# dog-qiuqiu/Yolo-FastestV2

Hardware: AMD Instinct MI355X
Metric: images/sec at 352x352 bs=256 per GPU (forward+decode+NMS) (higher is better)
Workload: dtype f32 tensors; contractions fp16x3 (two-term fp16 split operands on v_mfma_f32_16x16x32_f16, fp32 accumulate); depthwise/BN/ReLU/decode/NMS fp32 VALU; 1 GPU

## Files before the change

### include/yfv2.h

```cpp
#ifndef YFV2_H
#define YFV2_H

#include <stdint.h>

#ifdef __cplusplus
extern "C" {
#endif

#define YFV2_ABI_VERSION 7
#define YFV2_API __attribute__((visibility("default")))
#define YFV2_MAX_DET 300

typedef enum yfv2_status {
  YFV2_OK = 0,
  YFV2_ERR_ARG = -1,
  YFV2_ERR_CONFIG = -2,
  YFV2_ERR_DEVICE = -3,
  YFV2_ERR_WEIGHTS = -4,
  YFV2_ERR_STATE = -5,
  YFV2_ERR_BATCH = -6,
  YFV2_ERR_RANGE = -7
} yfv2_status;

typedef struct yfv2_ctx* yfv2_handle;
// ... 169 lines not shown

YFV2_API int yfv2_train_bind(yfv2_handle h, const yfv2_tensor_desc* tensors, int32_t n, const yfv2_tensor_desc* grads, int32_t ng);
YFV2_API int yfv2_train_forward(yfv2_handle h, const float* x, int32_t B, float* const out6[6], void* stream);
YFV2_API int yfv2_train_backward(yfv2_handle h, const float* const grad6[6], void* stream);
YFV2_API int yfv2_sgd_step(yfv2_handle h, float* param, const float* grad, float* momentum_buf, int64_t n, float lr, float momentum,
                           float weight_decay, int32_t first_step, void* stream);
typedef struct yfv2_sgd_item {
  float* param; const float* grad; float* momentum_buf;
  int64_t n;
  int32_t first_step; int32_t reserved;
} yfv2_sgd_item;
YFV2_API int yfv2_sgd_step_multi(yfv2_handle h, const yfv2_sgd_item* items, int32_t n_items, float lr, float momentum, float weight_decay,
                                 void* stream);


YFV2_API int32_t yfv2_num_rows(yfv2_handle h);
YFV2_API int32_t yfv2_num_stages(yfv2_handle h);

YFV2_API int yfv2_stage_info(yfv2_handle h, int32_t i, char* name, int32_t name_cap, double* flops_per_image,
                    double* bytes_per_image, double* external_bytes_per_image);
YFV2_API int yfv2_stage_kernel(yfv2_handle h, int32_t i, char* name, int32_t name_cap);

YFV2_API int yfv2_profile_forward(yfv2_handle h, const float* x, int32_t B, float* const out6[6], int32_t iters,
                         float* ms, void* stream);

YFV2_API int yfv2_clock_probe_begin(yfv2_handle h, int32_t workgroups, float milliseconds, int32_t busy, void* stream);
YFV2_API int yfv2_clock_probe_end(yfv2_handle h, double out[6], void* stream);

YFV2_API int yfv2_debug_repeat_step(yfv2_handle h, const float* x, int32_t B, float* const out6[6], int32_t step, int32_t iters, void* stream);

YFV2_API int yfv2_debug_post(yfv2_handle h, const float* const out6[6], int32_t B, float conf_thres, double iou_thres,
                             float* dets, int32_t* idx, int32_t* count, void* stream);

YFV2_API int64_t yfv2_debug_activation(yfv2_handle h, int32_t which, int32_t B, float* host_dst, int64_t cap);

YFV2_API int64_t yfv2_debug_train_relu_output(yfv2_handle h, const char* conv_name, float* host_dst, int64_t capacity);

YFV2_API int yfv2_debug_plan_dryrun(const yfv2_config* cfg, const yfv2_tensor_desc* tensors, int32_t n, int32_t* n_steps, int64_t* blob_floats);
YFV2_API int yfv2_debug_plan_dryrun_ex(const yfv2_config* cfg, const yfv2_plan* plan, const yfv2_tensor_desc* tensors, int32_t n, int32_t* n_steps,
                                       int64_t* blob_floats);
YFV2_API int64_t yfv2_debug_plan_image(const yfv2_config* cfg, const yfv2_tensor_desc* tensors, int32_t n, int32_t step, char* name,
                                       int32_t name_cap, float* dst, int64_t cap);
YFV2_API int64_t yfv2_debug_plan_image_ex(const yfv2_config* cfg, const yfv2_plan* plan, const yfv2_tensor_desc* tensors, int32_t n, int32_t step,
                                          char* name, int32_t name_cap, float* dst, int64_t cap);
YFV2_API int yfv2_debug_plan_c2_label(const yfv2_config* cfg, const yfv2_tensor_desc* tensors, int32_t n, int32_t* label);

#ifdef __cplusplus
}
#endif
#endif
```

### yolo_fastestv2_amd/_lib.py

```python
import ctypes as C
import os

_HERE = os.path.dirname(os.path.abspath(__file__))
LIB_PATH = os.environ.get("YFV2_LIB") or os.path.join(_HERE, "libyfv2.so")
ABI_VERSION = 7
MAX_DET = 300

OK, ERR_ARG, ERR_CONFIG, ERR_DEVICE, ERR_WEIGHTS, ERR_STATE, ERR_BATCH, ERR_RANGE = 0, -1, -2, -3, -4, -5, -6, -7


class Config(C.Structure):
    _fields_ = [("classes", C.c_int32), ("anchor_num", C.c_int32), ("height", C.c_int32), ("width", C.c_int32),
                ("anchors", C.c_double * 12), ("max_batch", C.c_int32), ("device", C.c_int32)]


class Plan(C.Structure):
    _fields_ = [("struct_size", C.c_int32), ("fp32_matrix", C.c_int32), ("layer_by_layer", C.c_int32), ("post_two_launches", C.c_int32),
                ("front_two_launches", C.c_int32), ("towers_unpaired", C.c_int32), ("lanes", C.c_int32), ("trace", C.c_int32), ("trace_step", C.c_int32)]


PLAN_FIELDS = ("fp32_matrix", "layer_by_layer", "post_two_launches", "front_two_launches", "towers_unpaired", "lanes", "trace", "trace_step")


def make_plan(plan=None):
# ... 108 lines not shown
    "yfv2_detect_frames_yuv": (C.c_int, [C.c_void_p, C.POINTER(FrameYuv), C.c_int32, C.c_float, C.c_double, C.c_void_p, C.c_void_p,
                                         C.c_void_p, C.c_void_p]),
    "yfv2_detect_tiled_yuv": (C.c_int, [C.c_void_p, C.POINTER(FrameYuv), C.c_int32, C.POINTER(Tile), C.c_int32, C.c_float, C.c_double, C.c_double,
                                        C.c_int32, C.c_int32, C.c_void_p, C.c_void_p, C.c_void_p, C.c_void_p]),
    "yfv2_train_batch_frames_u8": (C.c_int, [C.c_void_p, C.POINTER(Frame), C.c_int32, C.POINTER(C.c_float), C.POINTER(C.c_float), C.c_void_p, C.c_void_p]),
    "yfv2_train_batch_frames_yuv": (C.c_int, [C.c_void_p, C.POINTER(FrameYuv), C.c_int32, C.POINTER(C.c_float), C.POINTER(C.c_float), C.c_void_p, C.c_void_p]),
    "yfv2_export_maps": (C.c_int, [C.c_void_p, C.POINTER(C.c_void_p), C.c_int32, C.c_void_p, C.c_void_p, C.c_void_p]),
    "yfv2_deploy_post": (C.c_int, [C.c_void_p, C.c_void_p, C.c_void_p, C.c_int32, C.c_void_p, C.c_float, C.c_float, C.c_void_p, C.c_void_p,
                                   C.c_int32, C.c_void_p]),
    "yfv2_deploy_dropped": (C.c_int, [C.c_void_p, C.POINTER(C.c_int32), C.c_void_p]),
    "yfv2_detect_deploy_frames_u8": (C.c_int, [C.c_void_p, C.POINTER(Frame), C.c_int32, C.c_float, C.c_float, C.c_void_p, C.c_void_p,
                                               C.c_int32, C.c_void_p]),
    "yfv2_anchor_kmeans": (C.c_int, [C.c_void_p, C.c_void_p, C.c_int64, C.c_void_p, C.c_int32, C.c_int32, C.c_void_p, C.c_void_p,
                                     C.POINTER(KmeansInfo), C.c_void_p]),
    "yfv2_debug_kmeans_group": (C.c_int, [C.c_void_p, C.c_int32]),
    "yfv2_ap_per_class": (C.c_int, [C.c_void_p, C.c_void_p, C.c_void_p, C.c_void_p, C.c_int64, C.c_void_p, C.c_int64, C.POINTER(ApResult), C.c_void_p]),
    "yfv2_ap_per_class_multi": (C.c_int, [C.c_void_p, C.c_void_p, C.c_void_p, C.c_void_p, C.c_int64, C.c_void_p, C.c_int64, C.c_int32,
                                          C.POINTER(ApResult), C.c_void_p]),
    "yfv2_debug_plan_dryrun": (C.c_int, [C.c_void_p, C.c_void_p, C.c_int32, C.POINTER(C.c_int32), C.POINTER(C.c_int64)]),
    "yfv2_debug_plan_dryrun_ex": (C.c_int, [C.c_void_p, C.POINTER(Plan), C.c_void_p, C.c_int32, C.POINTER(C.c_int32), C.POINTER(C.c_int64)]),
    "yfv2_debug_plan_image": (C.c_int64, [C.c_void_p, C.c_void_p, C.c_int32, C.c_int32, C.c_char_p, C.c_int32, C.c_void_p, C.c_int64]),
    "yfv2_debug_plan_image_ex": (C.c_int64, [C.c_void_p, C.POINTER(Plan), C.c_void_p, C.c_int32, C.c_int32, C.c_char_p, C.c_int32, C.c_void_p, C.c_int64]),
    "yfv2_debug_plan_c2_label": (C.c_int, [C.c_void_p, C.c_void_p, C.c_int32, C.POINTER(C.c_int32)]),
    "yfv2_num_rows": (C.c_int32, [C.c_void_p]),
    "yfv2_num_stages": (C.c_int32, [C.c_void_p]),
    "yfv2_stage_info": (C.c_int, [C.c_void_p, C.c_int32, C.c_char_p, C.c_int32, C.POINTER(C.c_double),
                                  C.POINTER(C.c_double), C.POINTER(C.c_double)]),
    "yfv2_stage_kernel": (C.c_int, [C.c_void_p, C.c_int32, C.c_char_p, C.c_int32]),
    "yfv2_profile_forward": (C.c_int, [C.c_void_p, C.c_void_p, C.c_int32, C.POINTER(C.c_void_p), C.c_int32,
                                       C.POINTER(C.c_float), C.c_void_p]),
    "yfv2_debug_repeat_step": (C.c_int, [C.c_void_p, C.c_void_p, C.c_int32, C.POINTER(C.c_void_p), C.c_int32, C.c_int32, C.c_void_p]),
    "yfv2_debug_post": (C.c_int, [C.c_void_p, C.POINTER(C.c_void_p), C.c_int32, C.c_float, C.c_double, C.c_void_p, C.c_void_p,
                                  C.c_void_p, C.c_void_p]),
    "yfv2_debug_activation": (C.c_int64, [C.c_void_p, C.c_int32, C.c_int32, C.c_void_p, C.c_int64]),
    "yfv2_debug_train_relu_output": (C.c_int64, [C.c_void_p, C.c_char_p, C.c_void_p, C.c_int64]),
}

_lib = None


def lib():
    global _lib
    if _lib is not None:
        return _lib
    if not os.path.exists(LIB_PATH):
        raise ImportError("%s is missing: the HIP extension has not been built (run __graft_entry__.build()); "
                          "yolo_fastestv2_amd has no CPU or PyTorch fallback" % LIB_PATH)
    L = C.CDLL(LIB_PATH)
    if not hasattr(L, "yfv2_abi_version"):
        raise ImportError("%s does not export yfv2_abi_version: not a libyfv2 build" % LIB_PATH)
    L.yfv2_abi_version.restype, L.yfv2_abi_version.argtypes = C.c_int, []
    if L.yfv2_abi_version() != ABI_VERSION:
        raise ImportError("libyfv2.so ABI %d != binding ABI %d: rebuild (__graft_entry__.build())" % (L.yfv2_abi_version(), ABI_VERSION))
    for name, (res, args) in _PROTOTYPES.items():
        if name.startswith("yfv2_debug_") and os.environ.get("YFV2_LIB") and not hasattr(L, name):
            continue
        fn = getattr(L, name)
        fn.restype = res
        fn.argtypes = args
    _lib = L
    return L


def last_error(handle=None):
    msg = lib().yfv2_last_error(handle)
    return msg.decode("utf-8", "replace") if msg else ""
# ... 6 lines not shown
```

### yolo_fastestv2_amd/csrc/yfv2_api.hip

```cpp
#include <algorithm>
#include <cstdio>

#include "yfv2_ctx.h"

void read_plan_switches(yfv2_ctx* h, const yfv2_plan* plan) {
  h->sw.plan = read_sized(plan);
  h->sw.bf6 = !h->sw.plan.fp32_matrix;
  h->postfuse = !h->sw.plan.post_two_launches;
  h->sw.front_wanted = !h->sw.plan.front_two_launches;
}

int run_plan(yfv2_ctx* h, const void* x, bool x_u8, int B, float* const out6[6], hipStream_t stream, hipEvent_t* ev, int only_step) {
  const RunCtx c{h->d_params, x, x_u8, B, out6, stream, h->sw.bf6, h->nonfinite.dev};
  std::string err;
  if (int rc = plan_run(h->plan, c, h->d_trace, h->trace_step, ev, only_step, &err)) return fail(h, rc, err);
  if (only_step < 0) { h->last_x = x; h->last_B = B; h->last_u8 = x_u8; }
  HIP_TRY(h, hipGetLastError());
  return YFV2_OK;
}

int check_call(yfv2_ctx* h, int B, bool need_weights) {
  if (!h) return fail(nullptr, YFV2_ERR_ARG, "null handle");
  if (B < 1 || B > h->cfg.max_batch)
    return fail(h, YFV2_ERR_BATCH, "batch " + std::to_string(B) + " outside [1, max_batch=" + std::to_string(h->cfg.max_batch) + "]");
// ... 116 lines not shown
  return YFV2_OK;
}

void** yfv2_ctx_train_slot(yfv2_ctx* h) { return h ? &h->train : nullptr; }
const yfv2_config* yfv2_ctx_config(yfv2_ctx* h) { return &h->cfg; }
int yfv2_ctx_fail(yfv2_ctx* h, int code, const char* msg) {
  g_tls_error = msg ? msg : "";
  if (h) h->err = g_tls_error;
  return code;
}

DecodeArgs decode_args(yfv2_ctx* h, const float* const out6[6], int32_t B) {
  DecodeArgs a{};
  for (int sc = 0; sc < 2; ++sc) {
    a.reg[sc] = out6[sc * 3 + 0];
    a.obj[sc] = out6[sc * 3 + 1];
    a.cls[sc] = out6[sc * 3 + 2];
    a.fh[sc] = h->fh[sc];
    a.fw[sc] = h->fw[sc];
    a.stride[sc] = (float)((double)h->cfg.height / (double)h->fh[sc]);
  }
  for (int i = 0; i < 12; ++i) a.anchors[i] = h->cfg.anchors[i];
  a.B = B;
  a.classes = h->cfg.classes;
  a.rows = h->rows;
  return a;
}

NmsArgs nms_args(const yfv2_ctx* h, const float* boxes, int compact, int32_t B, float conf_thres, double iou_thres, float* dets, int32_t* idx, int32_t* count) {
  NmsArgs a{};
  a.boxes = boxes; a.compact = compact; a.dets = dets; a.idx = idx; a.count = count;
  a.B = B; a.rows = h->rows; a.nc = h->cfg.classes;
  a.conf_thres = conf_thres; a.iou_thres = iou_thres;
  return a;
}

static const void* image_at(const yfv2_ctx* h, const void* x, bool x_u8, int off) {
  return static_cast<const char*>(x) + (size_t)off * 3 * h->cfg.height * h->cfg.width * (x_u8 ? 1 : sizeof(float));
}

extern "C" {

int yfv2_abi_version(void) { return YFV2_ABI_VERSION; }

const char* yfv2_last_error(yfv2_handle h) { return h ? h->err.c_str() : g_tls_error.c_str(); }

int yfv2_create(yfv2_handle* out, const yfv2_config* cfg) { return yfv2_create_ex(out, cfg, nullptr); }

int yfv2_create_ex(yfv2_handle* out, const yfv2_config* cfg, const yfv2_plan* plan) {
  if (!out || !cfg) return fail(nullptr, YFV2_ERR_ARG, "yfv2_create: null argument");
  *out = nullptr;
  int rows = 0;
  if (int rc = check_config(cfg, &rows)) return rc;

  int ndev = 0;
  if (hipGetDeviceCount(&ndev) != hipSuccess || ndev <= 0 || cfg->device < 0 || cfg->device >= ndev)
    return fail(nullptr, YFV2_ERR_DEVICE, "no usable HIP device (this library has no CPU fallback)");
  hipDeviceProp_t prop;
  if (hipGetDeviceProperties(&prop, cfg->device) != hipSuccess)
    return fail(nullptr, YFV2_ERR_DEVICE, "hipGetDeviceProperties failed");
  if (std::strncmp(prop.gcnArchName, "gfx950", 6) != 0)
    return fail(nullptr, YFV2_ERR_DEVICE, std::string("device is ") + prop.gcnArchName + ", this library is built for gfx950 (MI355X) only");

  yfv2_ctx* h = new yfv2_ctx();
  h->in_lane = g_creating_lane;
  DeviceGuard guard(cfg->device);
// ... 244 lines not shown
```

### yolo_fastestv2_amd/csrc/yfv2_api_debug.hip

```cpp
#include <algorithm>
#include <cstdio>
#include <variant>

#include "yfv2_ctx.h"

namespace {

struct DryRun {
  yfv2_ctx ctx;
  WeightPacker wp;
  int build(const yfv2_config* cfg, const yfv2_plan* plan, const yfv2_tensor_desc* tensors, int32_t n) {
    int rows = 0;
    if (int rc = check_config(cfg, &rows)) return rc;
    uintptr_t next = 0x100000000ull;
    auto fake = [&](yfv2_ctx* hh, Buf* b, size_t per_img) {
      b->per_img = per_img;
      b->p = reinterpret_cast<float*>(next);
      next += (per_img * sizeof(float) * (size_t)hh->cfg.max_batch + 4095) & ~(uintptr_t)4095;
      return (int)YFV2_OK;
    };
    setup_ctx(&ctx, cfg, rows, fake);
    read_plan_switches(&ctx, plan);
    return build_plan(&ctx, wp, tensors, n, nullptr);
  }
};

}

extern "C" {

int yfv2_debug_plan_dryrun(const yfv2_config* cfg, const yfv2_tensor_desc* tensors, int32_t n, int32_t* n_steps, int64_t* blob_floats) {
  return yfv2_debug_plan_dryrun_ex(cfg, nullptr, tensors, n, n_steps, blob_floats);
}

int yfv2_debug_plan_dryrun_ex(const yfv2_config* cfg, const yfv2_plan* plan, const yfv2_tensor_desc* tensors, int32_t n, int32_t* n_steps, int64_t* blob_floats) {
  if (!cfg || !tensors || n <= 0) return fail(nullptr, YFV2_ERR_ARG, "yfv2_debug_plan_dryrun: bad argument");
  DryRun d;
  if (int rc = d.build(cfg, plan, tensors, n)) return rc;
  for (const Step& st : d.ctx.plan.steps)
    if (step_image(st) > d.wp.blob.size()) return fail(nullptr, YFV2_ERR_WEIGHTS, "step '" + st.name + "': image offset outside the blob");
  if (n_steps) *n_steps = (int32_t)d.ctx.plan.steps.size();
  if (blob_floats) *blob_floats = (int64_t)d.wp.blob.size();
  return YFV2_OK;
}

int64_t yfv2_debug_plan_image(const yfv2_config* cfg, const yfv2_tensor_desc* tensors, int32_t n, int32_t step, char* name, int32_t name_cap,
                              float* dst, int64_t cap) {
  return yfv2_debug_plan_image_ex(cfg, nullptr, tensors, n, step, name, name_cap, dst, cap);
}

int64_t yfv2_debug_plan_image_ex(const yfv2_config* cfg, const yfv2_plan* plan, const yfv2_tensor_desc* tensors, int32_t n, int32_t step, char* name,
                                 int32_t name_cap, float* dst, int64_t cap) {
  if (!cfg || !tensors || n <= 0 || (step != -1 && (!dst || cap <= 0))) return fail(nullptr, YFV2_ERR_ARG, "yfv2_debug_plan_image: bad argument");
  DryRun d;
  if (int rc = d.build(cfg, plan, tensors, n)) return rc;
  const int job = step >= 1000 ? step / 1000 - 1 : -1;
  if (step >= 1000) step %= 1000;
  std::vector<Step> view = d.ctx.plan.steps;
  if (d.ctx.plan.front_fused) { view.insert(view.begin(), d.ctx.plan.stem_aside); view[1].name = std::get<S2PxStep>(view[1].kind).name_plain; }
  if (step == -1) return (int64_t)view.size();
  if (step < 0 || step >= (int32_t)view.size()) return fail(nullptr, YFV2_ERR_ARG, "yfv2_debug_plan_image: step out of range");
  const TowerStep* tw = std::get_if<TowerStep>(&view[step].kind);
// ... 207 lines not shown
```

### yolo_fastestv2_amd/csrc/yfv2_internal.h

```cpp
#pragma once
#include <hip/hip_runtime.h>
#include <hip/hip_ext.h>
#include <stdint.h>

#include <atomic>

struct Yfv2LaunchProbe { hipEvent_t start = nullptr, stop = nullptr; int launches = 0; };
extern thread_local Yfv2LaunchProbe yfv2_launch_probe;
#define YFV2_LAUNCH(kernel, grid, block, lds, stream, ...)                                                                        \
  do {                                                                                                                             \
    Yfv2LaunchProbe& yfv2_lp_ = yfv2_launch_probe;                                                                                 \
    hipExtLaunchKernelGGL(kernel, grid, block, lds, stream, yfv2_lp_.launches++ == 0 ? yfv2_lp_.start : nullptr, yfv2_lp_.stop, 0, \
                          __VA_ARGS__);                                                                                            \
  } while (0)
struct Yfv2Device { int index, cus; };
inline Yfv2Device yfv2_device() {
  static std::atomic<int> cus_of[64];
  int dev = 0;
  if (hipGetDevice(&dev) != hipSuccess || dev < 0 || dev > 63) dev = 0;
  int cus = cus_of[dev].load(std::memory_order_relaxed);
  if (cus <= 0) { if (hipDeviceGetAttribute(&cus, hipDeviceAttributeMultiprocessorCount, dev) != hipSuccess || cus <= 0) cus = 256; cus_of[dev].store(cus, std::memory_order_relaxed); }
  return {dev, cus};
}
inline int yfv2_device_cus() { return yfv2_device().cus; }
// ... 162 lines not shown
  int B, H, W;
  long long* trace;
  int bf6;
  const float* img16;
  int chain;
  int* nonfinite;
};

struct DecodeArgs {
  const float* reg[2];
  const float* obj[2];
  const float* cls[2];
  float* boxes;
  float* cand;
  int B, classes;
  int fh[2], fw[2];
  float stride[2];
  double anchors[12];
  int rows;
};

struct NmsArgs {
  const float* boxes;
  int compact;
  float* dets;
  int32_t* idx;
  int32_t* count;
  const int32_t* classes;
  int n_classes;
  int B, rows, nc;
  float conf_thres;
  double iou_thres;
  long long* trace;
};

void yfv2_launch_stem(const StemArgs& a, hipStream_t s);
void yfv2_launch_stem16(const StemArgs& a, hipStream_t s);
bool yfv2_launch_pw(int K, int mode, const PwArgs& a, hipStream_t s);
int yfv2_pw_tiles(int K, int mode, int M);
bool yfv2_pw_presplit_supported(int K, int mode, int M);
bool yfv2_launch_dw(int ksize, int stride, const DwArgs& a, hipStream_t s);
int yfv2_block_s2_rows(int cin, int H, int W);
bool yfv2_launch_block_s2(int cin, const BlockS2Args& a, hipStream_t s);
bool yfv2_tower2_supported(int H, int W);
bool yfv2_launch_tower2(const TowerArgs& a, hipStream_t s);
bool yfv2_towerh_supported(int H, int W);
bool yfv2_towerh_multi(int H, int W);
bool yfv2_towerp_map(int H, int W);
void towerp_lane_patches(int H, int W, unsigned char (&tbl)[128]);
struct TowerJobs {
  TowerArgs j[4];
  int n;
  int par;
  int gpj;
  unsigned char lane_patch[128];
};
bool yfv2_launch_towerh(const TowerJobs& jobs, int mh_tiles, const Yfv2Device& dev, hipStream_t s);
struct StatsArgs {
  const float* dets;
  const int32_t* count;
  const float* targets;
  int32_t* tp;
  int32_t* overflow;
  int B, T;
  float iou_thres;
};
// ... 44 lines not shown
  double box_x, box_y;
};
void yfv2_launch_resize_frames(const ResizeFrame* frames, int B, int max_w, unsigned char* dst, int H, int W, hipStream_t s);
struct YuvCoef { int off, cy, cvr, cvg, cug, cub; };
struct ResizeFrameYuv {
  const unsigned char* y;
  const unsigned char* ca;
  const unsigned char* cb;
  long long pitch_y, pitch_c;
  int h, w;
  int px, py;
  int format;
  YuvCoef coef;
  double scale_x, scale_y;
};
size_t yfv2_resize_yuv_lds_bytes(int w, int W);
int yfv2_resize_yuv_max_width(int W);
YuvCoef yfv2_yuv_coef(int colour);
void yfv2_launch_resize_frames_yuv(const ResizeFrameYuv* frames, int B, int max_w, unsigned char* dst, int H, int W, hipStream_t s);
struct TrainFrame : ResizeFrame { float alpha, beta; };
struct TrainFrameYuv : ResizeFrameYuv { float alpha, beta; };
size_t yfv2_train_batch_lds_bytes(int SW, int W);
int yfv2_train_batch_max_width(int W);
size_t yfv2_train_batch_yuv_lds_bytes(int w, int W);
int yfv2_train_batch_yuv_max_width(int W);
void yfv2_launch_train_batch_frames(const TrainFrame* frames, int B, int max_w, float* dst , int H, int W, hipStream_t s);
void yfv2_launch_train_batch_frames_yuv(const TrainFrameYuv* frames, int B, int max_w, float* dst, int H, int W, hipStream_t s);
void yfv2_launch_frame_boxes(float* dets, const int32_t* count, const ResizeFrame* frames, int B, hipStream_t s);
void yfv2_launch_decode(const DecodeArgs& a, hipStream_t s);
void yfv2_launch_nms(const NmsArgs& a, hipStream_t s);
void yfv2_launch_decode_nms(const DecodeArgs& d, const NmsArgs& a, hipStream_t s);
bool yfv2_post_fusable(int classes, int rows);
int yfv2_nms_max_rows();
struct TileMergeArgs {
  const float* tile_dets;
  const int32_t* tile_count;
  const int32_t* table;
  int T, F;
  float* geo;
  float* meta;
  double thres;
  int metric;
  int max_out;
  float* dets;
  int32_t* src;
  int32_t* count;
};
void yfv2_launch_tile_merge(const TileMergeArgs& a, hipStream_t s);
struct ExportMapsArgs {
  const float* reg[2]; const float* obj[2]; const float* cls[2];
  float* map[2];
  int B, classes;
  int fh[2], fw[2];
};
void yfv2_launch_export_maps(const ExportMapsArgs& a, hipStream_t s);
struct DeployPostArgs {
  const float* map[2];
  const float* scale;
  int B, classes;
  int fh[2], fw[2];
  int stride[2];
  float anchors[12];
  int rows;
  float thresh, nms_thresh;
  int32_t* boxes;
  int32_t* count;
// ... 65 lines not shown
```

### yolo_fastestv2_amd/csrc/yfv2_post.hip

```cpp
#include "yfv2_device.h"


template <int J>
__device__ __forceinline__ int quad_xor(int v) {
  static_assert(J == 1 || J == 2, "quad_perm exchange inside four lanes");
  return __builtin_amdgcn_update_dpp(0, v, J == 1 ? 0xB1 : 0x4E, 0xF, 0xF, false);
}
template <int J> __device__ __forceinline__ float quad_xor(float v) { return __int_as_float(quad_xor<J>(__float_as_int(v))); }

template <bool SKIP = false, int MAXPER = 24>
__device__ __forceinline__ void yfv2_compact_row(const DecodeArgs& a, int b, int sc, int cc, int part, f32x4& r0, f32x4& r1,
                                                 float objl = 0.f, float skip_ct = 0.f) {
  const int fh = a.fh[sc], fw = a.fw[sc], hw = fh * fw;
  const int nc = a.classes;
  const int per = (nc + 3) >> 2;
  const int c_lo = part * per, c_hi = min(nc, c_lo + per);
  const int an = part < 3 ? part : 0;
  const float* cls = a.cls[sc] + (size_t)b * nc * hw;
  const float so = sigmoid_f32(SKIP ? objl : a.obj[sc][((size_t)b * 3 + an) * hw + cc]);
  float conf = 0.f;
  int cj = 0;
  int need = 1;
  if constexpr (SKIP) {
    need = so > skip_ct ? 1 : 0;
// ... 158 lines not shown
        float o[5];
        box_of(part, o);
        float* d = srow + part * rowlen;
#pragma unroll
        for (int k = 0; k < 5; ++k) d[k] = o[k];
      }
    }
    __syncthreads();
    float* dst = a.boxes + row0 * rowlen;
    const int n = ncell * 3 * rowlen;
    for (int i = tid; i < n; i += THREADS) dst[i] = stage[i];
  }
}

void yfv2_launch_decode(const DecodeArgs& a, hipStream_t s) {
  const int cells = a.classes <= 96 ? DEC_CELLS : 32;
  const int b0 = (a.fh[0] * a.fw[0] + cells - 1) / cells;
  const int b1 = (a.fh[1] * a.fw[1] + cells - 1) / cells;
  const size_t lds = (size_t)cells * 3 * (5 + a.classes) * sizeof(float);
  if (a.classes <= 96) {
    if (a.cand)
      YFV2_LAUNCH(decode_kernel<true>, dim3(a.B * (b0 + b1)), dim3(DEC_THREADS), 0, s, a, b0, b1);
    else
      YFV2_LAUNCH_LDS(yfv2_device(), decode_kernel<false>, YFV2_LDS_FULL, dim3(a.B * (b0 + b1)), dim3(DEC_THREADS), lds, s, a, b0, b1);
  } else {
    if (a.cand)
      YFV2_LAUNCH((decode_kernel<true, 64>), dim3(a.B * (b0 + b1)), dim3(4 * cells), 0, s, a, b0, b1);
    else
      YFV2_LAUNCH_LDS(yfv2_device(), (decode_kernel<false, 64>), YFV2_LDS_FULL, dim3(a.B * (b0 + b1)), dim3(4 * cells), lds, s, a, b0, b1);
  }
}
bool yfv2_post_fusable(int classes, int rows) { return classes <= 96 && rows <= 2048; }
int yfv2_nms_max_rows() { return 4096; }

constexpr int NMS_THREADS = 1024;
constexpr int NMS_NQ = NMS_THREADS / 64;
constexpr int NMS_CAP = 2048;
constexpr int NMS_MAX_DET = 300;

__device__ __forceinline__ unsigned xor_sel_mask() {
  const int l = (int)(threadIdx.x & 63);
  const bool s4 = __builtin_amdgcn_update_dpp(0, l, 0x124, 0xF, 0xF, false) == (l ^ 4);
  const auto p16 = __builtin_amdgcn_permlane16_swap(l, l, false, false);
  const auto p32 = __builtin_amdgcn_permlane32_swap(l, l, false, false);
  return (s4 ? 4u : 0u) | ((int)p16[0] == (l ^ 16) ? 16u : 0u) | ((int)p32[0] == (l ^ 32) ? 32u : 0u);
}
template <int J>
__device__ __forceinline__ unsigned xor_lane32(unsigned v, unsigned sel) {
  const int x = (int)v;
  if constexpr (J == 1 || J == 2) return (unsigned)quad_xor<J>(x);
  else if constexpr (J == 8) return (unsigned)__builtin_amdgcn_update_dpp(0, x, 0x128, 0xF, 0xF, false);
  else if constexpr (J == 4) {
    const int r4 = __builtin_amdgcn_update_dpp(0, x, 0x124, 0xF, 0xF, false), r12 = __builtin_amdgcn_update_dpp(0, x, 0x12C, 0xF, 0xF, false);
    return (unsigned)((sel & 4u) ? r4 : r12);
  } else if constexpr (J == 16) {
    const auto p = __builtin_amdgcn_permlane16_swap(x, x, false, false);
    return (unsigned)((sel & 16u) ? (int)p[0] : (int)p[1]);
  } else {
    static_assert(J == 32, "lane distance");
    const auto p = __builtin_amdgcn_permlane32_swap(x, x, false, false);
    return (unsigned)((sel & 32u) ? (int)p[0] : (int)p[1]);
  }
}
template <int J>
__device__ __forceinline__ unsigned long long xor_lane64(unsigned long long v, unsigned sel) {
  return ((unsigned long long)xor_lane32<J>((unsigned)(v >> 32), sel) << 32) | xor_lane32<J>((unsigned)v, sel);
}

template <int KPT>
__device__ __forceinline__ void bitonic_sort(unsigned long long* key, unsigned long long* key2, int np2, int tid) {
  const unsigned sel = xor_sel_mask();
// ... 36 lines not shown
      _Pragma("unroll") for (int r = 0; r < KPT; ++r) {                                     \
        const int i = tid + r * NMS_THREADS;                                                \
        k[r] = cx(k[r], xor_lane64<J>(k[r], sel), low == ((i & kk) == 0));                 \
      }                                                                                     \
    }
    YFV2_SORT_STEP(32) YFV2_SORT_STEP(16) YFV2_SORT_STEP(8) YFV2_SORT_STEP(4) YFV2_SORT_STEP(2) YFV2_SORT_STEP(1)
#undef YFV2_SORT_STEP
  }
  __syncthreads();
#pragma unroll
  for (int r = 0; r < KPT; ++r) { const int i = tid + r * NMS_THREADS; if (i < np2) key[i] = k[r]; }
  __syncthreads();
}

__device__ __forceinline__ unsigned conf_key(float c) {
  const unsigned u = __float_as_uint(c == 0.f ? 0.f : c);
  return (u & 0x80000000u) ? ~u : (u | 0x80000000u);
}

template <int SRC, int KPT = 2>
__global__ __launch_bounds__(NMS_THREADS) void nms_kernel(NmsArgs a, DecodeArgs dec) {
  constexpr bool COMPACT = SRC >= 1;
  constexpr int CAP = KPT * NMS_THREADS;
  static_assert(KPT == 2 || (KPT == 4 && SRC != 2), "two keys per thread, or four without the in-LDS decode");
  extern __shared__ __attribute__((aligned(16))) float crow[];
  __shared__ unsigned long long key[CAP];
  __shared__ __attribute__((aligned(16))) float geo[(KPT == 2 ? 7 : 5) * CAP];
  unsigned long long* const key2 = reinterpret_cast<unsigned long long*>(geo);
  float* const bx1 = geo + (KPT == 2 ? 2 * CAP : 0);
  float* const by1 = bx1 + CAP; float* const bx2 = by1 + CAP; float* const by2 = bx2 + CAP; float* const area = by2 + CAP;
  __shared__ unsigned char supp[CAP];
  __shared__ unsigned char cls_of_row[CAP];
  __shared__ int keep[NMS_MAX_DET];
  __shared__ float kx1[NMS_MAX_DET], kx2[NMS_MAX_DET];
  __shared__ unsigned long long pmask[NMS_NQ][64];
  __shared__ int n_cand, n_keep, n_obj;

  const int tid = threadIdx.x, b = blockIdx.x;
  const int rowlen = COMPACT ? 8 : 5 + a.nc;
  const float* img = SRC == 2 ? crow : a.boxes + (size_t)b * a.rows * rowlen;
  const float ct = a.conf_thres;
  YFV2_STAMP(0);
  if constexpr (SRC == 2) {
    constexpr int WC = 16;
    const int hw0 = dec.fh[0] * dec.fw[0], hw1 = dec.fh[1] * dec.fw[1];
    const int nw0 = (hw0 + WC - 1) / WC, nw = nw0 + (hw1 + WC - 1) / WC;
    const int wv = __builtin_amdgcn_readfirstlane(tid >> 6);
    const int part = tid & 3, an = part < 3 ? part : 0;
    auto obj_of = [&](int w) -> float {
      if (w >= nw) return 0.f;
      const int sc = w >= nw0 ? 1 : 0, hw = sc ? hw1 : hw0;
      const int cell = (w - (sc ? nw0 : 0)) * WC + ((tid & 63) >> 2);
      return dec.obj[sc][((size_t)b * 3 + an) * hw + (cell < hw ? cell : hw - 1)];
    };
    float ocur = obj_of(wv);
    for (int w = wv; w < nw; w += NMS_NQ) {
      const float onxt = obj_of(w + NMS_NQ);
      const int sc = w >= nw0 ? 1 : 0, hw = sc ? hw1 : hw0;
      const int row_base = sc ? 3 * hw0 : 0;
      const int cell = (w - (sc ? nw0 : 0)) * WC + ((tid & 63) >> 2);
      const bool ok = cell < hw;
      f32x4 r0, r1;
      yfv2_compact_row<true>(dec, b, sc, ok ? cell : hw - 1, part, r0, r1, ocur, ct);
      if (ok && part < 3) {
        float* d = crow + (size_t)(row_base + cell * 3 + part) * 8;
        *reinterpret_cast<f32x4*>(d) = r0;
        *reinterpret_cast<f32x4*>(d + 4) = r1;
// ... 70 lines not shown
    }
  }
  __syncthreads();
  YFV2_STAMP(2);
  const int n = n_cand;
  if (n == 0) {
    if (tid == 0) a.count[b] = 0;
    return;
  }

  int np2 = 1;
  while (np2 < n) np2 <<= 1;
  for (int i = n + tid; i < np2; i += NMS_THREADS) key[i] = 0ull;
  __syncthreads();
  if (np2 <= NMS_THREADS) bitonic_sort<1>(key, key2, np2, tid);
  else bitonic_sort<KPT>(key, key2, np2, tid);

  YFV2_STAMP(3);
  for (int i = tid; i < n; i += NMS_THREADS) {
    const unsigned row = 0xFFFFFFFFu - (unsigned)(key[i] & 0xFFFFFFFFull);
    const float* r = img + (size_t)row * rowlen;
    const float cx = r[0], cy = r[1], hw_ = __fdiv_rn(r[2], 2.0f), hh = __fdiv_rn(r[3], 2.0f);
    const float c = __fmul_rn((float)cls_of_row[row], 4096.0f);
    const float x1 = __fadd_rn(__fsub_rn(cx, hw_), c), y1 = __fadd_rn(__fsub_rn(cy, hh), c);
    const float x2 = __fadd_rn(__fadd_rn(cx, hw_), c), y2 = __fadd_rn(__fadd_rn(cy, hh), c);
    bx1[i] = x1; by1[i] = y1; bx2[i] = x2; by2[i] = y2;
    area[i] = __fmul_rn(__fsub_rn(x2, x1), __fsub_rn(y2, y1));
    supp[i] = 0;
  }
  __syncthreads();

  YFV2_STAMP(4);
  const bool thr_nonneg = a.iou_thres >= 0.0;
  auto overlaps = [&](int i, int j) -> bool {
    const float xx1 = fmaxf(bx1[i], bx1[j]), xx2 = fminf(bx2[i], bx2[j]);
    if (thr_nonneg && !(xx2 > xx1)) return false;
    const float yy1 = fmaxf(by1[i], by1[j]), yy2 = fminf(by2[i], by2[j]);
    const float w = fmaxf(0.0f, __fsub_rn(xx2, xx1)), h = fmaxf(0.0f, __fsub_rn(yy2, yy1));
    const float inter = __fmul_rn(w, h);
    const float ovr = __fdiv_rn(inter, __fsub_rn(__fadd_rn(area[i], area[j]), inter));
    return (double)ovr > a.iou_thres;
  };
  const int j = tid & 63, q = tid >> 6;
  long long t_tests = 0, t_walk = 0, t_bar = 0; int n_chunks = 0;
  const bool tr = a.trace && blockIdx.x == 0 && tid == 0;
  for (int c0 = 0; c0 < n; c0 += 64) {
    const int nk = n_keep;
    if (nk >= NMS_MAX_DET) break;
    const long long ts0 = tr ? (long long)__builtin_readcyclecounter() : 0;
    const int m = min(64, n - c0);
    unsigned long long bits = 0ull;
    {
      constexpr int KMAX = (NMS_MAX_DET + NMS_NQ - 1) / NMS_NQ;
      constexpr int PER = 64 / NMS_NQ;
      auto lane_f = [](float v, int l) { return __builtin_bit_cast(float, __builtin_amdgcn_readlane(__builtin_bit_cast(int, v), l)); };
      const int cj = c0 + j;
      const bool live = j < m;
      const float jx1 = live ? bx1[cj] : INFINITY, jx2 = live ? bx2[cj] : -INFINITY;
      const int kl = q + NMS_NQ * j;
      const bool kv = j < KMAX && kl < nk;
      const float rk1 = kv ? kx1[kl] : INFINITY, rk2 = kv ? kx2[kl] : -INFINITY;
      unsigned cand = 0u;
#pragma unroll
      for (int t = 0; t < KMAX; ++t) {
        const float a1 = lane_f(rk1, t), a2 = lane_f(rk2, t);
        if (q + NMS_NQ * t < nk && (!thr_nonneg || fminf(a2, jx2) > fmaxf(a1, jx1))) cand |= 1u << t;
      }
      unsigned icand = 0u;
#pragma unroll
      for (int c = 0; c < PER; ++c) {
        const int i = PER * q + c;
        const float a1 = lane_f(jx1, i), a2 = lane_f(jx2, i);
        if (i < j && (!thr_nonneg || fminf(a2, jx2) > fmaxf(a1, jx1))) icand |= 1u << c;
      }
      if (live) {
        while (cand) {
          const int t = __builtin_ctz(cand);
          cand &= cand - 1u;
          if (overlaps(keep[q + NMS_NQ * t], cj)) { supp[cj] = 1; break; }
        }
        while (icand) {
          const int c = __builtin_ctz(icand);
          icand &= icand - 1u;
          if (overlaps(c0 + PER * q + c, cj)) bits |= 1ull << (PER * q + c);
        }
      }
    }
    pmask[q][j] = bits;
    const long long ts1 = tr ? (long long)__builtin_readcyclecounter() : 0;
    __syncthreads();
    const long long ts2 = tr ? (long long)__builtin_readcyclecounter() : 0;
    if (tid < 64) {
      unsigned long long S = 0ull;
#pragma unroll
      for (int qq = 0; qq < NMS_NQ; ++qq) S |= pmask[qq][tid];
      const bool alive = tid < m && !supp[c0 + tid];
      const unsigned long long alive_mask = __ballot(alive);
      unsigned long long kmask = alive_mask;
      for (int it = 0; it < 64; ++it) {
        const unsigned long long k2 = __ballot(alive && !(S & kmask));
        if (k2 == kmask) break;
        kmask = k2;
      }
      if ((kmask >> tid) & 1ull) {
        const int pos = nk + __popcll(kmask & ((1ull << tid) - 1ull));
        if (pos < NMS_MAX_DET) { keep[pos] = c0 + tid; kx1[pos] = bx1[c0 + tid]; kx2[pos] = bx2[c0 + tid]; }
      }
      if (tid == 0) n_keep = min(NMS_MAX_DET, nk + __popcll(kmask));
    }
    const long long ts3 = tr ? (long long)__builtin_readcyclecounter() : 0;
    __syncthreads();
    if (tr) { const long long ts4 = (long long)__builtin_readcyclecounter(); t_tests += ts1 - ts0; t_walk += ts3 - ts2; t_bar += (ts2 - ts1) + (ts4 - ts3); ++n_chunks; }
  }
  if (tr) { a.trace[9] = n_chunks; a.trace[10] = t_tests; a.trace[11] = t_walk; a.trace[12] = t_bar; }
  __syncthreads();
  YFV2_STAMP(5);
  const int kept = n_keep;

  for (int k = tid; k < kept; k += NMS_THREADS) {
    const int i = keep[k];
    const unsigned long long kk = key[i];
    const unsigned row = 0xFFFFFFFFu - (unsigned)(kk & 0xFFFFFFFFull);
    const float* r = img + (size_t)row * rowlen;
    const float cx = r[0], cy = r[1], hw_ = __fdiv_rn(r[2], 2.0f), hh = __fdiv_rn(r[3], 2.0f);
    float* d = a.dets + ((size_t)b * NMS_MAX_DET + k) * 6;
    d[0] = __fsub_rn(cx, hw_); d[1] = __fsub_rn(cy, hh);
    d[2] = __fadd_rn(cx, hw_); d[3] = __fadd_rn(cy, hh);
    d[4] = COMPACT ? r[5] : __fmul_rn(r[5 + cls_of_row[row]], r[4]);
    d[5] = (float)cls_of_row[row];
    a.idx[(size_t)b * NMS_MAX_DET + k] = (int)row;
  }
  if (tid == 0) a.count[b] = kept;
  YFV2_STAMP(6);
  if (a.trace && blockIdx.x == 0 && tid == 0) { a.trace[7] = n; a.trace[8] = kept; }
}

void yfv2_launch_nms(const NmsArgs& a, hipStream_t s) {
  const DecodeArgs none{};
  if (a.rows <= NMS_CAP) {
// ... 170 lines not shown
```

Baseline: 463,400 images/s.

## Make NMS overlap tests wave-uniform with full kept-box arrays and a division-free reject

The NMS inner loop now keeps full kept-box coordinates and areas in LDS, laid out per wave, and tests them with wave-uniform scalar operands instead of divergent candidate walks. A conservative multiply-based test against a precomputed threshold skips the IoU division for pairs that clearly fall below the threshold. Within-chunk tests also compute full IoU for every lane instead of branching. The aim is to remove divergent loops and most divisions from the NMS critical path, at the cost of doing more uniform arithmetic per pair and a slightly larger LDS footprint.

```diff
diff --git a/include/yfv2.h b/include/yfv2.h
--- a/include/yfv2.h
+++ b/include/yfv2.h
@@ -225,6 +225,8 @@
 YFV2_API int yfv2_debug_post(yfv2_handle h, const float* const out6[6], int32_t B, float conf_thres, double iou_thres,
                              float* dets, int32_t* idx, int32_t* count, void* stream);
 
+YFV2_API int yfv2_debug_nms_reject(double iou_thres, float* c, float* c2);
+
 YFV2_API int64_t yfv2_debug_activation(yfv2_handle h, int32_t which, int32_t B, float* host_dst, int64_t cap);
 
 YFV2_API int64_t yfv2_debug_train_relu_output(yfv2_handle h, const char* conv_name, float* host_dst, int64_t capacity);
diff --git a/yolo_fastestv2_amd/_lib.py b/yolo_fastestv2_amd/_lib.py
--- a/yolo_fastestv2_amd/_lib.py
+++ b/yolo_fastestv2_amd/_lib.py
@@ -164,6 +164,7 @@
     "yfv2_debug_repeat_step": (C.c_int, [C.c_void_p, C.c_void_p, C.c_int32, C.POINTER(C.c_void_p), C.c_int32, C.c_int32, C.c_void_p]),
     "yfv2_debug_post": (C.c_int, [C.c_void_p, C.POINTER(C.c_void_p), C.c_int32, C.c_float, C.c_double, C.c_void_p, C.c_void_p,
                                   C.c_void_p, C.c_void_p]),
+    "yfv2_debug_nms_reject": (C.c_int, [C.c_double, C.POINTER(C.c_float), C.POINTER(C.c_float)]),
     "yfv2_debug_activation": (C.c_int64, [C.c_void_p, C.c_int32, C.c_int32, C.c_void_p, C.c_int64]),
     "yfv2_debug_train_relu_output": (C.c_int64, [C.c_void_p, C.c_char_p, C.c_void_p, C.c_int64]),
 }
diff --git a/yolo_fastestv2_amd/csrc/yfv2_api.hip b/yolo_fastestv2_amd/csrc/yfv2_api.hip
--- a/yolo_fastestv2_amd/csrc/yfv2_api.hip
+++ b/yolo_fastestv2_amd/csrc/yfv2_api.hip
@@ -172,6 +172,8 @@
   a.boxes = boxes; a.compact = compact; a.dets = dets; a.idx = idx; a.count = count;
   a.B = B; a.rows = h->rows; a.nc = h->cfg.classes;
   a.conf_thres = conf_thres; a.iou_thres = iou_thres;
+  float c;
+  a.rej_on = yfv2_nms_reject(iou_thres, &c, &a.rej_c2);
   return a;
 }
 
diff --git a/yolo_fastestv2_amd/csrc/yfv2_api_debug.hip b/yolo_fastestv2_amd/csrc/yfv2_api_debug.hip
--- a/yolo_fastestv2_amd/csrc/yfv2_api_debug.hip
+++ b/yolo_fastestv2_amd/csrc/yfv2_api_debug.hip
@@ -28,6 +28,14 @@
 }
 
 extern "C" {
+
+int yfv2_debug_nms_reject(double iou_thres, float* c, float* c2) {
+  float c_, c2_;
+  const int on = yfv2_nms_reject(iou_thres, &c_, &c2_);
+  if (c) *c = c_;
+  if (c2) *c2 = c2_;
+  return on;
+}
 
 int yfv2_debug_plan_dryrun(const yfv2_config* cfg, const yfv2_tensor_desc* tensors, int32_t n, int32_t* n_steps, int64_t* blob_floats) {
   return yfv2_debug_plan_dryrun_ex(cfg, nullptr, tensors, n, n_steps, blob_floats);
diff --git a/yolo_fastestv2_amd/csrc/yfv2_internal.h b/yolo_fastestv2_amd/csrc/yfv2_internal.h
--- a/yolo_fastestv2_amd/csrc/yfv2_internal.h
+++ b/yolo_fastestv2_amd/csrc/yfv2_internal.h
@@ -218,6 +218,8 @@
   float conf_thres;
   double iou_thres;
   long long* trace;
+  float rej_c2;
+  int rej_on;
 };
 
 void yfv2_launch_stem(const StemArgs& a, hipStream_t s);
@@ -328,6 +330,7 @@
 void yfv2_launch_decode_nms(const DecodeArgs& d, const NmsArgs& a, hipStream_t s);
 bool yfv2_post_fusable(int classes, int rows);
 int yfv2_nms_max_rows();
+int yfv2_nms_reject(double iou_thres, float* c, float* c2);
 struct TileMergeArgs {
   const float* tile_dets;
   const int32_t* tile_count;
diff --git a/yolo_fastestv2_amd/csrc/yfv2_post.hip b/yolo_fastestv2_amd/csrc/yfv2_post.hip
--- a/yolo_fastestv2_amd/csrc/yfv2_post.hip
+++ b/yolo_fastestv2_amd/csrc/yfv2_post.hip
@@ -214,11 +214,22 @@
 }
 bool yfv2_post_fusable(int classes, int rows) { return classes <= 96 && rows <= 2048; }
 int yfv2_nms_max_rows() { return 4096; }
+int yfv2_nms_reject(double iou_thres, float* c, float* c2) {
+  *c = 0.f; *c2 = 0.f;
+  if (!(iou_thres >= 0x1p-24 && iou_thres <= 1.0)) return 0;
+  auto fp32_at_most = [](double v) { float f = (float)v; return (double)f > v ? nextafterf(f, -INFINITY) : f; };
+  *c = fp32_at_most(iou_thres);
+  *c2 = fp32_at_most((double)*c * (1.0 - 0x1p-22));
+  return 1;
+}
 
 constexpr int NMS_THREADS = 1024;
 constexpr int NMS_NQ = NMS_THREADS / 64;
 constexpr int NMS_CAP = 2048;
 constexpr int NMS_MAX_DET = 300;
+#ifndef YFV2_NMS_UNIFORM
+#define YFV2_NMS_UNIFORM 1
+#endif
 
 __device__ __forceinline__ unsigned xor_sel_mask() {
   const int l = (int)(threadIdx.x & 63);
@@ -321,7 +332,8 @@
   __shared__ unsigned char supp[CAP];
   __shared__ unsigned char cls_of_row[CAP];
   __shared__ int keep[NMS_MAX_DET];
-  __shared__ float kx1[NMS_MAX_DET], kx2[NMS_MAX_DET];
+  constexpr int KMAX = (NMS_MAX_DET + NMS_NQ - 1) / NMS_NQ;
+  __shared__ float kx1[NMS_NQ * KMAX], ky1[NMS_NQ * KMAX], kx2[NMS_NQ * KMAX], ky2[NMS_NQ * KMAX], karea[NMS_NQ * KMAX];
   __shared__ unsigned long long pmask[NMS_NQ][64];
   __shared__ int n_cand, n_keep, n_obj;
 
@@ -458,59 +470,92 @@
 
   YFV2_STAMP(4);
   const bool thr_nonneg = a.iou_thres >= 0.0;
-  auto overlaps = [&](int i, int j) -> bool {
-    const float xx1 = fmaxf(bx1[i], bx1[j]), xx2 = fminf(bx2[i], bx2[j]);
-    if (thr_nonneg && !(xx2 > xx1)) return false;
-    const float yy1 = fmaxf(by1[i], by1[j]), yy2 = fminf(by2[i], by2[j]);
+  const bool rej_on = a.rej_on != 0;
+  const float rej_c2 = a.rej_c2;
+  auto vmax = [](auto a, float m) -> float {
+    float r;
+    if constexpr (__is_same(decltype(a), int)) asm("v_max_f32 %0, %1, %2" : "=v"(r) : "s"(a), "v"(m));
+    else asm("v_max_f32 %0, %1, %2" : "=v"(r) : "v"(a), "v"(m));
+    return r;
+  };
+  auto vmin = [](auto a, float m) -> float {
+    float r;
+    if constexpr (__is_same(decltype(a), int)) asm("v_min_f32 %0, %1, %2" : "=v"(r) : "s"(a), "v"(m));
+    else asm("v_min_f32 %0, %1, %2" : "=v"(r) : "v"(a), "v"(m));
+    return r;
+  };
+  auto pair = [&](auto ax1, auto ay1, auto ax2, auto ay2, float aarea, float mx1, float my1, float mx2, float my2, float marea, float& inter, float& uni) {
+    const float xx1 = vmax(ax1, mx1), xx2 = vmin(ax2, mx2);
+    const float yy1 = vmax(ay1, my1), yy2 = vmin(ay2, my2);
     const float w = fmaxf(0.0f, __fsub_rn(xx2, xx1)), h = fmaxf(0.0f, __fsub_rn(yy2, yy1));
-    const float inter = __fmul_rn(w, h);
-    const float ovr = __fdiv_rn(inter, __fsub_rn(__fadd_rn(area[i], area[j]), inter));
-    return (double)ovr > a.iou_thres;
+    inter = __fmul_rn(w, h);
+    uni = __fsub_rn(__fadd_rn(aarea, marea), inter);
   };
-  const int j = tid & 63, q = tid >> 6;
+  auto rejected = [&](float inter, float uni) -> bool { return rej_on && uni >= 0x1p-100f && uni < INFINITY && inter < __fmul_rn(rej_c2, uni); };
+  auto above = [&](float inter, float uni) -> bool { return (double)__fdiv_rn(inter, uni) > a.iou_thres; };
+  const int j = tid & 63, q = __builtin_amdgcn_readfirstlane(tid >> 6);
   long long t_tests = 0, t_walk = 0, t_bar = 0; int n_chunks = 0;
   const bool tr = a.trace && blockIdx.x == 0 && tid == 0;
   for (int c0 = 0; c0 < n; c0 += 64) {
-    const int nk = n_keep;
+    const int nk = __builtin_amdgcn_readfirstlane(n_keep);
     if (nk >= NMS_MAX_DET) break;
     const long long ts0 = tr ? (long long)__builtin_readcyclecounter() : 0;
     const int m = min(64, n - c0);
     unsigned long long bits = 0ull;
-    {
-      constexpr int KMAX = (NMS_MAX_DET + NMS_NQ - 1) / NMS_NQ;
-      constexpr int PER = 64 / NMS_NQ;
-      auto lane_f = [](float v, int l) { return __builtin_bit_cast(float, __builtin_amdgcn_readlane(__builtin_bit_cast(int, v), l)); };
-      const int cj = c0 + j;
-      const bool live = j < m;
-      const float jx1 = live ? bx1[cj] : INFINITY, jx2 = live ? bx2[cj] : -INFINITY;
-      const int kl = q + NMS_NQ * j;
-      const bool kv = j < KMAX && kl < nk;
-      const float rk1 = kv ? kx1[kl] : INFINITY, rk2 = kv ? kx2[kl] : -INFINITY;
-      unsigned cand = 0u;
-#pragma unroll
-      for (int t = 0; t < KMAX; ++t) {
-        const float a1 = lane_f(rk1, t), a2 = lane_f(rk2, t);
-        if (q + NMS_NQ * t < nk && (!thr_nonneg || fminf(a2, jx2) > fmaxf(a1, jx1))) cand |= 1u << t;
-      }
-      unsigned icand = 0u;
-#pragma unroll
-      for (int c = 0; c < PER; ++c) {
-        const int i = PER * q + c;
-        const float a1 = lane_f(jx1, i), a2 = lane_f(jx2, i);
-        if (i < j && (!thr_nonneg || fminf(a2, jx2) > fmaxf(a1, jx1))) icand |= 1u << c;
-      }
-      if (live) {
-        while (cand) {
-          const int t = __builtin_ctz(cand);
+    constexpr int PER = 64 / NMS_NQ;
+    auto lane_i = [](float v, int l) { return __builtin_amdgcn_readlane(__builtin_bit_cast(int, v), l); };
+    auto lane_f = [&](float v, int l) { return __builtin_bit_cast(float, lane_i(v, l)); };
+    const int cj = c0 + j;
+    const bool live = j < m;
+    const float jx1 = live ? bx1[cj] : INFINITY, jx2 = live ? bx2[cj] : -INFINITY;
+    const float jy1 = live ? by1[cj] : 0.f, jy2 = live ? by2[cj] : 0.f, jarea = live ? area[cj] : 0.f;
+    const int ks = q * KMAX + j;
+    const bool kv = j < KMAX && q + NMS_NQ * j < nk;
+    const float rk1 = kv ? kx1[ks] : INFINITY, rk2 = kv ? kx2[ks] : -INFINITY;
+    bool open = live;
+#if YFV2_NMS_UNIFORM
+    const float rky1 = kv ? ky1[ks] : 0.f, rky2 = kv ? ky2[ks] : 0.f, rka = kv ? karea[ks] : 0.f;
+    const int nt = q < nk ? (nk - q + NMS_NQ - 1) / NMS_NQ : 0;
+#pragma unroll 1
+    for (int t = 0; t < nt; ++t) {
+      float inter, uni;
+      pair(lane_i(rk1, t), lane_i(rky1, t), lane_i(rk2, t), lane_i(rky2, t), lane_f(rka, t), jx1, jy1, jx2, jy2, jarea, inter, uni);
+      if (open && !rejected(inter, uni) && above(inter, uni)) open = false;
+    }
+#else
+    auto xmeet = [&](float ax1, float ax2, float mx1, float mx2) -> bool { return !thr_nonneg || fminf(ax2, mx2) > fmaxf(ax1, mx1); };
+    unsigned cand = 0u;
+#pragma unroll
+    for (int t = 0; t < KMAX; ++t) {
+      const float a1 = lane_f(rk1, t), a2 = lane_f(rk2, t);
+      if (live && q + NMS_NQ * t < nk && xmeet(a1, a2, jx1, jx2)) cand |= 1u << t;
+    }
+    if (cand) {
+      int s = q * KMAX + __builtin_ctz(cand);
+      cand &= cand - 1u;
+      float n0 = kx1[s], n1 = ky1[s], n2 = kx2[s], n3 = ky2[s], n4 = karea[s];
+      for (;;) {
+        const float e0 = n0, e1 = n1, e2 = n2, e3 = n3, e4 = n4;
+        const bool more = cand != 0u;
+        if (more) {
+          s = q * KMAX + __builtin_ctz(cand);
           cand &= cand - 1u;
-          if (overlaps(keep[q + NMS_NQ * t], cj)) { supp[cj] = 1; break; }
-        }
-        while (icand) {
-          const int c = __builtin_ctz(icand);
-          icand &= icand - 1u;
-          if (overlaps(c0 + PER * q + c, cj)) bits |= 1ull << (PER * q + c);
-        }
-      }
+          n0 = kx1[s]; n1 = ky1[s]; n2 = kx2[s]; n3 = ky2[s]; n4 = karea[s];
+        }
+        float inter, uni;
+        pair(e0, e1, e2, e3, e4, jx1, jy1, jx2, jy2, jarea, inter, uni);
+        if (!rejected(inter, uni) && above(inter, uni)) { open = false; break; }
+        if (!more) break;
+      }
+    }
+#endif
+    if (live && !open) supp[cj] = 1;
+#pragma unroll
+    for (int c = 0; c < PER; ++c) {
+      const int i = PER * q + c;
+      float inter, uni;
+      pair(lane_i(jx1, i), lane_i(jy1, i), lane_i(jx2, i), lane_i(jy2, i), lane_f(jarea, i), jx1, jy1, jx2, jy2, jarea, inter, uni);
+      if (open && i < j && !rejected(inter, uni) && above(inter, uni)) bits |= 1ull << i;
     }
     pmask[q][j] = bits;
     const long long ts1 = tr ? (long long)__builtin_readcyclecounter() : 0;
@@ -530,7 +575,10 @@
       }
       if ((kmask >> tid) & 1ull) {
         const int pos = nk + __popcll(kmask & ((1ull << tid) - 1ull));
-        if (pos < NMS_MAX_DET) { keep[pos] = c0 + tid; kx1[pos] = bx1[c0 + tid]; kx2[pos] = bx2[c0 + tid]; }
+        if (pos < NMS_MAX_DET) {
+          const int s = (pos % NMS_NQ) * KMAX + pos / NMS_NQ;
+          keep[pos] = cj; kx1[s] = jx1; ky1[s] = jy1; kx2[s] = jx2; ky2[s] = jy2; karea[s] = jarea;
+        }
       }
       if (tid == 0) n_keep = min(NMS_MAX_DET, nk + __popcll(kmask));
     }
```

Result: no change. 466,800 images/s (median of 6 runs) (+0.7%).
